# zir-vision/ProbPose_pytorch

Measured on AMD Instinct MI355X. Metric: person_crops_per_sec, higher is better.
Workload: dtype bf16

## Files before the change

### include/probpose_hip.h

```cpp
#ifndef PROBPOSE_HIP_H
#define PROBPOSE_HIP_H

#include <stddef.h>
#include <stdint.h>

#ifdef __cplusplus
extern "C" {
#endif

#define PP_F32 0
#define PP_BF16 1
#define PP_FP8 2

#define PP_MAX_RADIUS 9
#define PP_MAX_TAPS (2 * PP_MAX_RADIUS + 1)

#define PP_EPI_BIAS 1
#define PP_EPI_GELU 2
#define PP_EPI_RELU 4
#define PP_EPI_RESIDUAL 8
#define PP_EPI_OUT_F32 16
#define PP_EPI_ROWBIAS 32
#define PP_EPI_ROWSTATS 128
#define PP_EPI_LNFOLD 256
#define PP_EPI_OUT_FP8 512
#define PP_EPI_NOCLAMP 1024
#define PP_EPI_FUSE_FINAL 2048
#define PP_EPI_HEADMAJOR 4096
#define PP_EPI_HEATMAP 64

int pp_version(void);
const char *pp_last_error(void);
int pp_device_ok(void);

#define PP_DECODE_NO_WAVE 1
#define PP_DECODE_SCREEN 2
#define PP_DECODE_ALL_PIXEL 4
#define PP_DECODE_WAVE 16
size_t pp_decode_workspace_bytes(int B, int K, int H, int W);
int pp_decode_f32(const float *heatmaps, const float *prob, const float *vis,
                  const float *oks, const float *err, int B, int K, int H, int W,
                  const double *taps, const int *radius, double den_x, double den_y,
                  double in_w, double in_h, double *out_kpts, float *out_scores,
                  float *out_locs, float *out_aux, double *out_err, float *out_conv,
                  double *out_packed, void *workspace, int flags, void *stream);

typedef struct pp_gemm_args {
  const void *A; const void *W; void *C;
  const float *bias;
  const float *residual;
  const float *rowbias;
  const int32_t *rowoff;
  const int32_t *out_rowmap;
  int M, N, Kd;
  int lda, ldw, ldc;
  int seg_len;
  int rowbias_period;
  int batch;
  long long strideA, strideW, strideC, strideBias, strideRowoff, strideRowmap;
  int dtype;
  int epilogue;
  int hm_K, hm_HW;
  float hm_temperature;
  void *C2;
  int ldc2;
  float *stats_out;
  const float *stats_in;
  int stats_parts;
  const float *colsum;
  float ln_eps;
  int tile;
  float out_scale;
  int splitk;
  long long strideA_k, strideW_k, strideC_k, strideRowoff_k;
  const void *final_w;
  const float *final_b;
} pp_gemm_args;
int pp_gemm(const pp_gemm_args *args, void *stream);

int pp_layernorm(const float *x, const float *gamma, const float *beta, float eps,
                 int rows, int C, void *out, int dtype, void *stream);
int pp_layernorm_fp8(const float *x, const float *gamma, const float *beta, float eps,
                     int rows, int C, unsigned char *out, float inv_scale, void *stream);

int pp_attention(const void *qkv, void *out, int B, int N, int heads, int hd,
                 int dtype, void *stream);
int pp_attention_headmajor(const void *qkv, void *out, int B, int N, int heads, int hd, void *stream);
int pp_attention_fp8out(const void *qkv, unsigned char *out, int B, int N, int heads, int hd,
                        float inv_scale, void *stream);

int pp_qkv_attention_bf16(const void *h, const void *w_hm, const float *b_hm, void *out, int B, int heads, int C,
                          void *stream);

int pp_patchify(const float *x, void *out, int B, int H, int W, int patch, int dtype,
                void *stream);

int pp_maxpool_relu_sum(const float *x, int nsplit, long long split_stride, const float *bias, void *out, int B, int h,
                        int w, int C, int kh, int kw, int dtype, void *stream);

int pp_maxpool_relu(const void *x, void *out, int B, int h, int w, int C, int kh, int kw,
                    int dtype, void *stream);

int pp_final_heatmap(const void *x, const void *w, const float *bias, float *out, int B, int HW,
                     int Cin, int K, float temperature, int dtype, void *stream);

int pp_final_logits(const void *x, const void *w, const float *bias, float *out, int B, int HW,
                    int Cin, int K, float temperature, int dtype, void *stream);

int pp_sparsemax_rows(float *x, long long rows, int n, float scale, void *stream);

size_t pp_dark_decode_lds_bytes(int H, int W, int ksize);
int pp_dark_decode_f32(const float *heatmaps, int B, int K, int H, int W, const float *taps_host, int ksize,
                       double in_w, double in_h, double *out_kpts, float *out_scores, float *out_locs, void *stream);

int pp_aux_tail(const void *x, const void *w, const float *bias, float *out, int B, int C,
                int K, int dtype, void *stream);

int pp_tokens_to_nchw(const void *x, float *out, int B, int N, int C, int dtype, void *stream);
int pp_nchw_to_tokens(const float *x, void *out, int B, int C, int HW, int dtype, void *stream);

long long pp_frontend_plan_bytes(int n_boxes, const int *boxes_xyxy, int out_w, int out_h);
int pp_frontend_plan_build(int n_boxes, const int *boxes_xyxy, int out_w, int out_h, void *plan,
                           int *n_blocks_out, long long *lds_bytes_out);
int pp_frontend_crop_resize(const unsigned char *image, int img_w, int img_h, long long img_stride,
                            const void *plan_dev, int n_boxes, int n_blocks, long long lds_bytes,
                            int out_w, int out_h, float *out, void *stream);

#define PP_FRONTEND_SRC_ALIGN 4
#define PP_FRONTEND_SRC_PAD 4
long long pp_frontend_multi_plan_bytes(int n_boxes, const int *boxes_xyxy, int out_w, int out_h);
int pp_frontend_multi_plan_build(int n_boxes, const int *boxes_xyxy, const long long *sources, long long src_bytes,
                                 int out_w, int out_h, void *plan, int *n_blocks_out, long long *lds_bytes_out);
int pp_frontend_crop_resize_multi(const unsigned char *src, const void *plan_dev, int n_boxes, int n_blocks,
                                  long long lds_bytes, int out_w, int out_h, float *out, void *stream);

int pp_dataset_ground_truth(const float *kpts_raw, const double *boxes_xywh, int B, int K, int in_w, int in_h,
                            float scale_x, float scale_y, float *kpts_crop, float *kpts_hm, float *encode_visible,
                            unsigned char *in_image, unsigned char *keypoints_visible, float *keypoints_visibility,
                            void *stream);

int pp_augment_check(int n, const long long *sources, long long src_bytes, const double *warp,
                     const float *kp_affine, int K, const int *perm);
int pp_augment_warp(const unsigned char *src, const long long *sources, const double *warp, int n, int in_w,
                    int in_h, float *out, void *stream);
int pp_dataset_ground_truth_affine(const float *kpts_raw, const float *kp_affine, const int *perm, int B, int K,
                                   int in_w, int in_h, float scale_x, float scale_y, float *kpts_crop,
                                   float *kpts_hm, float *encode_visible, unsigned char *in_image,
                                   unsigned char *keypoints_visible, float *keypoints_visibility, void *stream);

#define PP_AUGMENT_POST_TILE_W 64
#define PP_AUGMENT_POST_TILE_H 16
int pp_augment_post_check(int n, const int *records, int in_w, int in_h, int filters);
int pp_augment_post(const float *in, const int *records, int n, int in_w, int in_h, int filters, float *out,
                    void *stream);

int pp_hflip_pair(const float *x, float *out, int B, int C, int H, int W, void *stream);
int pp_flip_merge(const float *heat2, const float *aux2, const int *perm, int B, int K, int H, int W,
                  float *heat_out, float *aux_out, void *stream);

int pp_encode_probmaps(const float *kpts_hm, const float *visible, const double *two_s, int B, int K, int H,
                       int W, float *heatmaps, float *weights, void *stream);

int pp_heatmap_argmax(const float *heatmaps, long long maps, int H, int W, float *locs, float *vals, void *stream);
int pp_pck_counts(const void *pred, const void *gt, int coord_f64, const unsigned char *mask, const double *norm,
                  const unsigned char *skip, double thr, int N, int K, int *counts, float *dist, void *stream);

// ... 222 lines not shown
```

### probpose_pytorch_amd/_lib.py

```python
from __future__ import annotations

import ctypes as C
import os
import threading

import numpy as np
import torch

_HERE = os.path.dirname(os.path.abspath(__file__))
LIB_PATH = os.path.join(_HERE, "lib", "libprobpose_hip.so")

PP_F32, PP_BF16, PP_FP8 = 0, 1, 2
PP_MAX_RADIUS = 9
PP_MAX_TAPS = 2 * PP_MAX_RADIUS + 1
EPI_BIAS, EPI_GELU, EPI_RELU, EPI_RESIDUAL, EPI_OUT_F32, EPI_ROWBIAS, EPI_HEATMAP = 1, 2, 4, 8, 16, 32, 64
DECODE_NO_WAVE, DECODE_SCREEN, DECODE_ALL_PIXEL, DECODE_WAVE = 1, 2, 4, 16
EPI_HEADMAJOR = 4096
EPI_OUT_FP8, EPI_NOCLAMP, EPI_FUSE_FINAL = 512, 1024, 2048

_lock = threading.Lock()
_lib = None


class HipExtensionError(RuntimeError):
    pass


class GemmArgs(C.Structure):
    _fields_ = [
        ("A", C.c_void_p), ("W", C.c_void_p), ("C", C.c_void_p),
        ("bias", C.c_void_p), ("residual", C.c_void_p), ("rowbias", C.c_void_p),
        ("rowoff", C.c_void_p), ("out_rowmap", C.c_void_p),
        ("M", C.c_int), ("N", C.c_int), ("Kd", C.c_int),
        ("lda", C.c_int), ("ldw", C.c_int), ("ldc", C.c_int),
        ("seg_len", C.c_int), ("rowbias_period", C.c_int), ("batch", C.c_int),
        ("strideA", C.c_longlong), ("strideW", C.c_longlong), ("strideC", C.c_longlong),
        ("strideBias", C.c_longlong), ("strideRowoff", C.c_longlong), ("strideRowmap", C.c_longlong),
        ("dtype", C.c_int), ("epilogue", C.c_int),
        ("hm_K", C.c_int), ("hm_HW", C.c_int), ("hm_temperature", C.c_float),
        ("C2", C.c_void_p), ("ldc2", C.c_int), ("stats_out", C.c_void_p), ("stats_in", C.c_void_p),
        ("stats_parts", C.c_int), ("colsum", C.c_void_p), ("ln_eps", C.c_float), ("tile", C.c_int),
        ("out_scale", C.c_float),
        ("splitk", C.c_int),
        ("strideA_k", C.c_longlong), ("strideW_k", C.c_longlong), ("strideC_k", C.c_longlong),
        ("strideRowoff_k", C.c_longlong),
        ("final_w", C.c_void_p), ("final_b", C.c_void_p),
    ]


class WgradArgs(C.Structure):
    _fields_ = [
        ("dY", C.c_void_p), ("dy_rowmap", C.c_void_p), ("ldd", C.c_longlong),
        ("A", C.c_void_p), ("rowoff", C.c_void_p), ("seg_len", C.c_int), ("lda", C.c_int),
        ("dW", C.c_void_p), ("lddw", C.c_longlong),
        ("dB", C.c_void_p),
        ("parts", C.c_void_p),
        ("M", C.c_int), ("N", C.c_int), ("Kd", C.c_int), ("batch", C.c_int),
        ("strideDY", C.c_longlong), ("strideA", C.c_longlong), ("strideRowoff", C.c_longlong),
        ("strideRowmap", C.c_longlong), ("strideDW", C.c_longlong), ("strideDB", C.c_longlong),
        ("dtype", C.c_int),
    ]


_vp, _i, _f, _d = C.c_void_p, C.c_int, C.c_float, C.c_double
_SIGNATURES = {
    "pp_version": (C.c_int, []),
    "pp_last_error": (C.c_char_p, []),
    "pp_device_ok": (C.c_int, []),
    "pp_decode_workspace_bytes": (C.c_size_t, [_i, _i, _i, _i]),
    "pp_decode_f32": (C.c_int, [_vp] * 5 + [_i] * 4 + [_vp, _vp] + [_d] * 4 + [_vp] * 8 + [_i, _vp]),
    "pp_gemm": (C.c_int, [C.POINTER(GemmArgs), _vp]),
    "pp_layernorm": (C.c_int, [_vp, _vp, _vp, _f, _i, _i, _vp, _i, _vp]),
    "pp_layernorm_fp8": (C.c_int, [_vp, _vp, _vp, _f, _i, _i, _vp, _f, _vp]),
    "pp_attention": (C.c_int, [_vp, _vp, _i, _i, _i, _i, _i, _vp]),
    "pp_attention_headmajor": (C.c_int, [_vp, _vp, _i, _i, _i, _i, _vp]),
    "pp_attention_fp8out": (C.c_int, [_vp, _vp, _i, _i, _i, _i, _f, _vp]),
    "pp_qkv_attention_bf16": (C.c_int, [_vp, _vp, _vp, _vp, _i, _i, _i, _vp]),
    "pp_patchify": (C.c_int, [_vp, _vp, _i, _i, _i, _i, _i, _vp]),
    "pp_maxpool_relu": (C.c_int, [_vp, _vp, _i, _i, _i, _i, _i, _i, _i, _vp]),
    "pp_maxpool_relu_sum": (C.c_int, [_vp, _i, C.c_longlong, _vp, _vp, _i, _i, _i, _i, _i, _i, _i, _vp]),
    "pp_final_heatmap": (C.c_int, [_vp, _vp, _vp, _vp, _i, _i, _i, _i, _f, _i, _vp]),
    "pp_final_logits": (C.c_int, [_vp, _vp, _vp, _vp, _i, _i, _i, _i, _f, _i, _vp]),
    "pp_sparsemax_rows": (C.c_int, [_vp, C.c_longlong, _i, _f, _vp]),
    "pp_dark_decode_lds_bytes": (C.c_size_t, [_i, _i, _i]),
    "pp_dark_decode_f32": (C.c_int, [_vp, _i, _i, _i, _i, _vp, _i, _d, _d, _vp, _vp, _vp, _vp]),
    "pp_aux_tail": (C.c_int, [_vp, _vp, _vp, _vp, _i, _i, _i, _i, _vp]),
    "pp_tokens_to_nchw": (C.c_int, [_vp, _vp, _i, _i, _i, _i, _vp]),
    "pp_nchw_to_tokens": (C.c_int, [_vp, _vp, _i, _i, _i, _i, _vp]),
    "pp_encode_probmaps": (C.c_int, [_vp, _vp, _vp, _i, _i, _i, _i, _vp, _vp, _vp]),
    "pp_heatmap_argmax": (C.c_int, [_vp, C.c_longlong, _i, _i, _vp, _vp, _vp]),
    "pp_pck_counts": (C.c_int, [_vp, _vp, _i, _vp, _vp, _vp, _d, _i, _i, _vp, _vp, _vp]),
    "pp_frontend_plan_bytes": (C.c_longlong, [_i, _vp, _i, _i]),
    "pp_frontend_plan_build": (C.c_int, [_i, _vp, _i, _i, _vp, C.POINTER(C.c_int), C.POINTER(C.c_longlong)]),
    "pp_frontend_crop_resize": (C.c_int, [_vp, _i, _i, C.c_longlong, _vp, _i, _i, C.c_longlong, _i, _i, _vp, _vp]),
    "pp_frontend_multi_plan_bytes": (C.c_longlong, [_i, _vp, _i, _i]),
    "pp_frontend_multi_plan_build": (C.c_int, [_i, _vp, _vp, C.c_longlong, _i, _i, _vp, C.POINTER(C.c_int),
                                               C.POINTER(C.c_longlong)]),
    "pp_frontend_crop_resize_multi": (C.c_int, [_vp, _vp, _i, _i, C.c_longlong, _i, _i, _vp, _vp]),
    "pp_dataset_ground_truth": (C.c_int, [_vp, _vp, _i, _i, _i, _i, _f, _f] + [_vp] * 7),
    "pp_augment_check": (C.c_int, [_i, _vp, C.c_longlong, _vp, _vp, _i, _vp]),
    "pp_augment_warp": (C.c_int, [_vp, _vp, _vp, _i, _i, _i, _vp, _vp]),
    "pp_dataset_ground_truth_affine": (C.c_int, [_vp, _vp, _vp, _i, _i, _i, _i, _f, _f] + [_vp] * 7),
    "pp_augment_post_check": (C.c_int, [_i, _vp, _i, _i, _i]),
    "pp_augment_post": (C.c_int, [_vp, _vp, _i, _i, _i, _i, _vp, _vp]),
    "pp_hflip_pair": (C.c_int, [_vp, _vp, _i, _i, _i, _i, _vp]),
    "pp_flip_merge": (C.c_int, [_vp, _vp, _vp, _i, _i, _i, _i, _vp, _vp, _vp]),
    "pp_oks_heatmap_loss": (C.c_int, [_vp, _vp, _vp, _i, _vp, C.c_longlong, C.c_longlong, _i, _i] + [_f] * 4
                            + [_i] * 4 + [_vp] * 5),
    "pp_probpose_loss_terms": (C.c_int, [_vp] * 10 + [_d, _i, _i, _i] + [_vp] * 6),
    "pp_oks_heatmap_loss_backward": (C.c_int, [_vp, _vp, _vp, _i, _vp, C.c_longlong, C.c_longlong, _i, _i]
                                     + [_f] * 4 + [_i, _vp] + [C.c_longlong] * 4 + [_i] * 4 + [_vp, _vp]),
    "pp_probpose_loss_grads": (C.c_int, [_vp] * 13 + [_i, _i] + [_vp] * 5),
    "pp_wgrad_workspace_floats": (C.c_longlong, [_i, _i, _i, _i]),
    "pp_wgrad_gemm": (C.c_int, [C.POINTER(WgradArgs), _vp]),
    "pp_bn_workspace_bytes": (C.c_longlong, [_i, _i]),
    "pp_bn_train_stats": (C.c_int, [_vp, C.c_longlong, _i, _i, _vp, _vp, _f, _f] + [_vp] * 8),
    "pp_bn_apply_relu": (C.c_int, [_vp, C.c_longlong, _i, _i, _vp, _vp, _vp, C.c_longlong, _i, _i, _vp]),
    "pp_bn_pool_relu": (C.c_int, [_vp, _i, _i, _i, _i, _i, _i, _vp, _vp, _vp, _vp, _i, _vp]),
    "pp_bn_train_backward": (C.c_int, [_vp, C.c_longlong, _vp, C.c_longlong, _i, _i] + [_vp] * 5
                             + [_i, _vp, _i, _i, _i, _i, _i, _vp, _vp, _vp, C.c_longlong, _i, _vp, _vp]),
    "pp_aux_tail_backward": (C.c_int, [_vp] * 4 + [_i, _i, _i] + [_vp] * 3 + [_i, _vp]),
    "pp_heat_clamp": (C.c_int, [_vp, _vp, C.c_longlong, _f, _vp]),
    "pp_heat_tail_backward": (C.c_int, [_vp, _vp, _i, _i, _i, _f, _i, _f, _vp, _i, _i, _vp]),
    "pp_layernorm_backward_workspace_bytes": (C.c_longlong, [_i, _i]),
    "pp_layernorm_backward": (C.c_int, [_vp, _vp, _f, _i, _i, _vp, C.c_longlong, _vp, _i, _vp, _i, _vp, _vp, _vp, _vp]),
    "pp_gelu_forward": (C.c_int, [_vp, C.c_longlong, _vp, _i, _vp]),
    "pp_gelu_backward": (C.c_int, [_vp, _vp, C.c_longlong, _vp, _i, _vp]),
    "pp_attention_backward_workspace_bytes": (C.c_longlong, [_i, _i, _i]),
    "pp_attention_backward": (C.c_int, [_vp] * 4 + [_i] * 5 + [_vp, _vp]),
    "pp_rows_period_sum": (C.c_int, [_vp, _i, _i, _i, _vp, _vp]),
    "pp_crop_rows_gather": (C.c_int, [_vp, _vp, _i, _i, _i, _i, _f, _vp, _i, _vp]),
    "pp_droppath_add": (C.c_int, [_vp, _vp, _vp, _i, _i, _i, _i, _f, _vp, _vp]),
    "pp_crop_rows_scatter_add": (C.c_int, [_vp, _vp, _i, _i, _i, _i, _vp, _vp, _i, _vp]),
    "pp_optim_table_bytes": (C.c_longlong, [_i, _vp, _i]),
    "pp_optim_table_build": (C.c_int, [_i] + [_vp] * 7 + [_i] + [_vp] * 3 + [_i, C.POINTER(C.c_int),
                                                                             C.POINTER(C.c_longlong)]),
    "pp_grad_sqnorm_partials": (C.c_int, [_vp, _i, _vp, _vp]),
    "pp_grad_norm_finish": (C.c_int, [_vp, _i, _i, _d, _i, _vp, _vp]),
    "pp_adamw_step": (C.c_int, [_vp, _i, _vp, _i, _vp]),
    "pp_ema_table_bytes": (C.c_longlong, [_i, _vp]),
    "pp_ema_table_build": (C.c_int, [_i] + [_vp] * 5 + [C.POINTER(C.c_int)]),
    "pp_ema_update": (C.c_int, [_vp, _i, _d, _vp]),
    "pp_cocoeval_oks": (C.c_int, [_i, _i] + [C.c_longlong] * 3 + [_vp] * 10),
    "pp_cocoeval_exoks": (C.c_int, [_i, _i] + [C.c_longlong] * 3 + [_vp] * 10 + [_d, _vp, _vp]),
    "pp_cocoeval_match": (C.c_int, [_i, _i, _i] + [C.c_longlong] * 3 + [_vp] * 13),
    "pp_cocoeval_accumulate": (C.c_int, [C.c_longlong, _i, _i, _i] + [_vp] * 10),
    "pp_posenms_rescore": (C.c_int, [C.c_longlong, _i, _vp, _vp, _d, _vp, _vp]),
    "pp_posenms": (C.c_int, [_i, _i, C.c_longlong] + [_vp] * 7 + [_i, _d, _d, _i] + [_vp] * 4),
    "pp_track_state_bytes": (C.c_longlong, [_i, _i]),
    "pp_track_oks": (C.c_int, [_i, _i, _i, C.c_longlong] + [_vp] * 7 + [_d, _vp, _vp]),
    "pp_track_assign": (C.c_int, [_i, _i, _i, C.c_longlong] + [_vp] * 5 + [_d, _i, _d, _d] + [_vp] * 6),
    "pp_track_assign_optimal": (C.c_int, [_i, _i, _i, C.c_longlong] + [_vp] * 5 + [_d, _i, _d, _d] + [_vp] * 7),
    "pp_track_oks_predicted": (C.c_int, [_i, _i, _i, C.c_longlong] + [_vp] * 7 + [_d, _d, _d, _vp, _vp]),
    "pp_track_assign_staged": (C.c_int, [_i, _i, _i, C.c_longlong] + [_vp] * 6 + [_d, _d, _d, _i, _d, _i, _i, _d, _d]
                               + [_vp] * 7),
    "pp_track_filter": (C.c_int, [_i, _i, C.c_longlong] + [_vp] * 4 + [_d] + [_vp] * 3 + [_i, _d, _d, _d, _vp, _vp]),
# ... 91 lines not shown
```

### probpose_pytorch_amd/csrc/pp_ops.hip

```cpp
#include <algorithm>

#include "pp_common.h"

namespace pp {

__device__ __forceinline__ float ln_sum4(float4 v) { return (v.x + v.y) + (v.z + v.w); }
__device__ __forceinline__ float ln_sqsum4(float4 v, float mean) {
  const float a = v.x - mean, b = v.y - mean, cc = v.z - mean, d = v.w - mean;
  return (a * a + b * b) + (cc * cc + d * d);
}
template <typename T>
__global__ __launch_bounds__(256) void layernorm_kernel(const float *__restrict__ x,
                                                        const float *__restrict__ gamma,
                                                        const float *__restrict__ beta, float eps,
                                                        int rows, int C, T *__restrict__ out, float qscale = 1.0f) {
  const int lane = threadIdx.x & 63;
  const int row = blockIdx.x * 4 + (threadIdx.x >> 6);
  if (row >= rows) return;
  const float *xr = x + (size_t)row * C;
  T *orow = out + (size_t)row * C;
  constexpr int MAXV = 8;
  if ((C & 3) == 0 && C <= MAXV * 256) {
    float4 v[MAXV];
    float s = 0.f;
#pragma unroll
    for (int i = 0; i < MAXV; ++i) {
      const int c = (i * 64 + lane) * 4;
      if (c < C) {
        v[i] = *reinterpret_cast<const float4 *>(xr + c);
        s += ln_sum4(v[i]);
      }
    }
    const float mean = wave_sum(s) / (float)C;
    float q = 0.f;
#pragma unroll
    for (int i = 0; i < MAXV; ++i) {
      const int c = (i * 64 + lane) * 4;
      if (c < C) {
        q += ln_sqsum4(v[i], mean);
      }
    }
    const float rstd = 1.0f / sqrtf(wave_sum(q) / (float)C + eps);
#pragma unroll
    for (int i = 0; i < MAXV; ++i) {
      const int c = (i * 64 + lane) * 4;
      if (c < C) {
        const float4 g = *reinterpret_cast<const float4 *>(gamma + c);
        const float4 b = *reinterpret_cast<const float4 *>(beta + c);
        const float o0 = (v[i].x - mean) * rstd * g.x + b.x, o1 = (v[i].y - mean) * rstd * g.y + b.y,
                    o2 = (v[i].z - mean) * rstd * g.z + b.z, o3 = (v[i].w - mean) * rstd * g.w + b.w;
        if constexpr (sizeof(T) == 4) {
          *reinterpret_cast<float4 *>(orow + c) = make_float4(o0, o1, o2, o3);
        } else if constexpr (sizeof(T) == 1) {
          *reinterpret_cast<unsigned *>(orow + c) = pack_fp8x4(o0 * qscale, o1 * qscale, o2 * qscale, o3 * qscale);
        } else {
          ushort4 pk;
          pk.x = f32_to_bf16(o0); pk.y = f32_to_bf16(o1); pk.z = f32_to_bf16(o2); pk.w = f32_to_bf16(o3);
          *reinterpret_cast<ushort4 *>(orow + c) = pk;
        }
      }
    }
    return;
  }
  float s = 0.f;
  for (int c = lane; c < C; c += 64) s += xr[c];
  const float mean = wave_sum(s) / (float)C;
  float q = 0.f;
  for (int c = lane; c < C; c += 64) {
    const float d = xr[c] - mean;
    q += d * d;
  }
  const float rstd = 1.0f / sqrtf(wave_sum(q) / (float)C + eps);
  if constexpr (sizeof(T) != 1)
    for (int c = lane; c < C; c += 64) Store<T>::st(orow + c, (xr[c] - mean) * rstd * gamma[c] + beta[c]);
}

template <typename T, int RPW, int NV>
__global__ __launch_bounds__(256) void layernorm_rows_kernel(const float *__restrict__ x,
                                                             const float *__restrict__ gamma,
                                                             const float *__restrict__ beta, float eps, int rows,
                                                             int C, T *__restrict__ out, float qscale) {
  const int lane = threadIdx.x & 63;
  const int row0 = (blockIdx.x * 4 + (threadIdx.x >> 6)) * RPW;
  if (row0 >= rows) return;
  float4 v[RPW][NV];
#pragma unroll
  for (int r = 0; r < RPW; ++r) {
    const float *xr = x + (size_t)min(row0 + r, rows - 1) * C;
#pragma unroll
    for (int i = 0; i < NV; ++i) {
      const int c = (i * 64 + lane) * 4;
      if (c < C) v[r][i] = *reinterpret_cast<const float4 *>(xr + c);
    }
  }
  float4 g[NV], bt[NV];
#pragma unroll
  for (int i = 0; i < NV; ++i) {
    const int c = (i * 64 + lane) * 4;
    if (c < C) {
      g[i] = *reinterpret_cast<const float4 *>(gamma + c);
      bt[i] = *reinterpret_cast<const float4 *>(beta + c);
    }
  }
#pragma unroll
  for (int r = 0; r < RPW; ++r) {
    float s = 0.f;
#pragma unroll
    for (int i = 0; i < NV; ++i) {
      const int c = (i * 64 + lane) * 4;
      if (c < C) s += ln_sum4(v[r][i]);
    }
    const float mean = wave_sum(s) / (float)C;
    float q = 0.f;
#pragma unroll
    for (int i = 0; i < NV; ++i) {
      const int c = (i * 64 + lane) * 4;
      if (c < C) {
        q += ln_sqsum4(v[r][i], mean);
      }
    }
    const float rstd = 1.0f / sqrtf(wave_sum(q) / (float)C + eps);
    if (row0 + r >= rows) continue;
    T *orow = out + (size_t)(row0 + r) * C;
#pragma unroll
    for (int i = 0; i < NV; ++i) {
      const int c = (i * 64 + lane) * 4;
      if (c < C) {
        const float o0 = (v[r][i].x - mean) * rstd * g[i].x + bt[i].x, o1 = (v[r][i].y - mean) * rstd * g[i].y + bt[i].y,
                    o2 = (v[r][i].z - mean) * rstd * g[i].z + bt[i].z, o3 = (v[r][i].w - mean) * rstd * g[i].w + bt[i].w;
        if constexpr (sizeof(T) == 4) {
          *reinterpret_cast<float4 *>(orow + c) = make_float4(o0, o1, o2, o3);
        } else if constexpr (sizeof(T) == 1) {
          *reinterpret_cast<unsigned *>(orow + c) = pack_fp8x4(o0 * qscale, o1 * qscale, o2 * qscale, o3 * qscale);
        } else {
          ushort4 pk;
          pk.x = f32_to_bf16(o0); pk.y = f32_to_bf16(o1); pk.z = f32_to_bf16(o2); pk.w = f32_to_bf16(o3);
          *reinterpret_cast<ushort4 *>(orow + c) = pk;
        }
      }
    }
  }
}

template <typename T>
static bool layernorm_rows_launch(const float *x, const float *gamma, const float *beta, float eps, int rows, int C,
                                  T *out, float qscale, hipStream_t s) {
  if ((C & 3) != 0 || C > 1280 || C <= 512 || rows < 2048) return false;
  const int want = (rows + 4095) / 4096;
  const int rpw = want >= 3 ? 3 : (want >= 2 ? 2 : 1);
  const int grid = cdiv(rows, 4 * rpw);
#define PP_LN_ROWS(RPW_, NV_)                                                                                     \
  hipLaunchKernelGGL((layernorm_rows_kernel<T, RPW_, NV_>), dim3(grid), dim3(256), 0, s, x, gamma, beta, eps, rows, C, \
                     out, qscale)
  if (C <= 768) {
    if (rpw == 3) PP_LN_ROWS(3, 3); else if (rpw == 2) PP_LN_ROWS(2, 3); else PP_LN_ROWS(1, 3);
  } else {
    if (rpw == 3) PP_LN_ROWS(3, 5); else if (rpw == 2) PP_LN_ROWS(2, 5); else PP_LN_ROWS(1, 5);
  }
#undef PP_LN_ROWS
  return true;
}

template <typename T>
__global__ __launch_bounds__(256) void patchify_kernel(const float *__restrict__ x, T *__restrict__ out,
                                                       int B, int H, int W, int p) {
  const int W4 = W >> 2;
  const long long total = (long long)B * 3 * H * W4;
  const int gw = W / p, gh = H / p;
  for (long long i = (long long)blockIdx.x * 256 + threadIdx.x; i < total; i += (long long)gridDim.x * 256) {
    const int xq = (int)(i % W4);
    long long t = i / W4;
    const int y = (int)(t % H);
    t /= H;
    const int c = (int)(t % 3);
    const int b = (int)(t / 3);
    const int x0 = xq * 4;
    const int gy = y / p, py = y - gy * p, gx = x0 / p, px = x0 - gx * p;
    if (gy >= gh || gx >= gw) continue;
    const float4 v = *reinterpret_cast<const float4 *>(x + (((size_t)b * 3 + c) * H + y) * W + x0);
    T *o = out + ((size_t)(b * gh + gy) * gw + gx) * (3 * p * p) + (c * p + py) * p + px;
    Store<T>::st(o + 0, v.x); Store<T>::st(o + 1, v.y); Store<T>::st(o + 2, v.z); Store<T>::st(o + 3, v.w);
  }
}

template <typename T>
__global__ __launch_bounds__(256) void maxpool_relu_kernel(const T *__restrict__ x, T *__restrict__ out,
                                                           int B, int h, int w, int C, int kh, int kw) {
  constexpr int VEC = 16 / (int)sizeof(T);
  const int oh = h / kh, ow = w / kw, CV = C / VEC;
  const long long total = (long long)B * oh * ow * CV;
  for (long long i = (long long)blockIdx.x * 256 + threadIdx.x; i < total; i += (long long)gridDim.x * 256) {
    const int cv = (int)(i % CV);
    long long t = i / CV;
    const int ox = (int)(t % ow);
    t /= ow;
    const int oy = (int)(t % oh);
    const int b = (int)(t / oh);
    float m[VEC];
#pragma unroll
    for (int e = 0; e < VEC; ++e) m[e] = 0.f;
    for (int dy = 0; dy < kh; ++dy)
      for (int dx = 0; dx < kw; ++dx) {
        const T *src = x + (((size_t)b * h + oy * kh + dy) * w + ox * kw + dx) * C + cv * VEC;
        const uint4 raw = *reinterpret_cast<const uint4 *>(src);
        const T *e8 = reinterpret_cast<const T *>(&raw);
#pragma unroll
        for (int e = 0; e < VEC; ++e) {
          const float f = Store<T>::ld(e8 + e);
          m[e] = (f > m[e] || f != f) ? f : m[e];
        }
      }
    uint4 pk;
    T *o8 = reinterpret_cast<T *>(&pk);
#pragma unroll
    for (int e = 0; e < VEC; ++e) Store<T>::st(o8 + e, m[e]);
    *reinterpret_cast<uint4 *>(out + (((size_t)b * oh + oy) * ow + ox) * C + cv * VEC) = pk;
  }
}

template <typename T>
__global__ __launch_bounds__(256) void maxpool_relu_sum_kernel(const float *__restrict__ x, int nsplit,
                                                               long long split_stride, const float *__restrict__ bias,
                                                               T *__restrict__ out, int B, int h, int w, int C, int kh,
                                                               int kw) {
  const int oh = h / kh, ow = w / kw, CV = C / 4;
  const long long total = (long long)B * oh * ow * CV;
  for (long long i = (long long)blockIdx.x * 256 + threadIdx.x; i < total; i += (long long)gridDim.x * 256) {
    const int cv = (int)(i % CV);
    long long t = i / CV;
    const int ox = (int)(t % ow);
    t /= ow;
    const int oy = (int)(t % oh);
    const int b = (int)(t / oh);
    const float4 bv = *reinterpret_cast<const float4 *>(bias + cv * 4);
    float m[4] = {0.f, 0.f, 0.f, 0.f};
    for (int dy = 0; dy < kh; ++dy)
      for (int dx = 0; dx < kw; ++dx) {
        const float *src = x + (((size_t)b * h + oy * kh + dy) * w + ox * kw + dx) * C + cv * 4;
        float4 a = *reinterpret_cast<const float4 *>(src);
        for (int sp = 1; sp < nsplit; ++sp) {
          const float4 q = *reinterpret_cast<const float4 *>(src + (size_t)sp * split_stride);
          a.x += q.x; a.y += q.y; a.z += q.z; a.w += q.w;
        }
        const float f[4] = {a.x + bv.x, a.y + bv.y, a.z + bv.z, a.w + bv.w};
#pragma unroll
        for (int e = 0; e < 4; ++e) m[e] = (f[e] > m[e] || f[e] != f[e]) ? f[e] : m[e];
      }
    T *o = out + (((size_t)b * oh + oy) * ow + ox) * C + cv * 4;
    if constexpr (sizeof(T) == 4) {
      *reinterpret_cast<float4 *>(o) = make_float4(m[0], m[1], m[2], m[3]);
    } else {
      ushort4 pk;
      pk.x = f32_to_bf16(m[0]); pk.y = f32_to_bf16(m[1]); pk.z = f32_to_bf16(m[2]); pk.w = f32_to_bf16(m[3]);
      *reinterpret_cast<ushort4 *>(o) = pk;
    }
  }
}

template <typename T>
__global__ __launch_bounds__(256) void aux_tail_kernel(const T *__restrict__ x, const T *__restrict__ w,
                                                       const float *__restrict__ bias,
                                                       float *__restrict__ out, int B, int C, int K,
                                                       int nbr, unsigned relu_mask) {
  const int lane = threadIdx.x & 63;
// ... 206 lines not shown
              const float4 kv = kr[d4];
              a = fmaf(q[4 * d4 + 0], kv.x, a);
              a = fmaf(q[4 * d4 + 1], kv.y, a);
              a = fmaf(q[4 * d4 + 2], kv.z, a);
              a = fmaf(q[4 * d4 + 3], kv.w, a);
            }
          } else {
            a = -__builtin_inff();
          }
          s[u] = a;
          gm = fmaxf(gm, a);
        }
        const float mn = fmaxf(m, gm);
        const float alpha = expf(m - mn);
        l *= alpha;
#pragma unroll
        for (int d = 0; d < HD; ++d) o[d] *= alpha;
#pragma unroll
        for (int u = 0; u < 8; ++u) {
          if (g + u < kc) {
            const float pu = expf(s[u] - mn);
            l += pu;
            const float4 *vr = reinterpret_cast<const float4 *>(Vs + (size_t)(g + u) * HD);
#pragma unroll
            for (int d4 = 0; d4 < HD / 4; ++d4) {
              const float4 vv = vr[d4];
              o[4 * d4 + 0] = fmaf(pu, vv.x, o[4 * d4 + 0]);
              o[4 * d4 + 1] = fmaf(pu, vv.y, o[4 * d4 + 1]);
              o[4 * d4 + 2] = fmaf(pu, vv.z, o[4 * d4 + 2]);
              o[4 * d4 + 3] = fmaf(pu, vv.w, o[4 * d4 + 3]);
            }
          }
        }
        m = mn;
      }
    }
    if (active) {
      const float inv = 1.0f / l;
      T *orow = out + ((size_t)b * N + qi) * C + h * HD;
#pragma unroll
      for (int d = 0; d < HD; ++d) Store<T>::st(orow + d, o[d] * inv);
    }
  }
}

template <typename T, int HD>
static int launch_attention_valu(const void *qkv, void *out, int B, int N, int heads, hipStream_t s) {
  int KC = (64 * 1024) / (2 * HD * 4);
  KC = (KC / 8) * 8;
  if (KC > N) KC = ((N + 7) / 8) * 8;
  const size_t lds = (size_t)2 * KC * HD * 4;
  int threads = ((N + 63) / 64) * 64;
  if (threads > 256) threads = 256;
  const float scale = 1.0f / sqrtf((float)HD);
  hipLaunchKernelGGL((attention_valu_kernel<T, HD>), dim3(B * heads), dim3(threads), lds, s,
                     (const T *)qkv, (T *)out, N, heads, scale, KC);
  PP_CHECK_LAUNCH("attention_valu_kernel");
  return 0;
}

template <typename T>
int attention_valu(const void *qkv, void *out, int B, int N, int heads, int hd, hipStream_t s) {
  switch (hd) {
    case 32: return launch_attention_valu<T, 32>(qkv, out, B, N, heads, s);
    case 64: return launch_attention_valu<T, 64>(qkv, out, B, N, heads, s);
    case 80: return launch_attention_valu<T, 80>(qkv, out, B, N, heads, s);
    default: return fail("pp_attention: head_dim %d not supported (32, 64, 80)", hd);
  }
}
template int attention_valu<float>(const void *, void *, int, int, int, int, hipStream_t);
template int attention_valu<bf16_t>(const void *, void *, int, int, int, int, hipStream_t);

static int grid_for(long long work_items) {
  long long g = (work_items + 255) / 256;
  if (g > 8192) g = 8192;
  if (g < 1) g = 1;
  return (int)g;
}

}

using namespace pp;

extern "C" int pp_layernorm(const float *x, const float *gamma, const float *beta, float eps, int rows,
                            int C, void *out, int dtype, void *stream) {
  PP_REQUIRE(rows >= 0 && C > 0, "pp_layernorm: bad shape");
  if (rows == 0) return 0;
  PP_REQUIRE(x && gamma && beta && out, "pp_layernorm: null pointer");
  hipStream_t s = (hipStream_t)stream;
  const int grid = cdiv(rows, 4);
  if (dtype == PP_BF16) {
    if (!layernorm_rows_launch<bf16_t>(x, gamma, beta, eps, rows, C, (bf16_t *)out, 1.0f, s))
      hipLaunchKernelGGL(layernorm_kernel<bf16_t>, dim3(grid), dim3(256), 0, s, x, gamma, beta, eps, rows, C,
                         (bf16_t *)out);
  } else if (dtype == PP_F32) {
    if (!layernorm_rows_launch<float>(x, gamma, beta, eps, rows, C, (float *)out, 1.0f, s))
      hipLaunchKernelGGL(layernorm_kernel<float>, dim3(grid), dim3(256), 0, s, x, gamma, beta, eps, rows, C,
                         (float *)out);
  } else {
    return fail("pp_layernorm: bad dtype %d", dtype);
  }
  PP_CHECK_LAUNCH("layernorm_kernel");
  return 0;
}

extern "C" int pp_layernorm_fp8(const float *x, const float *gamma, const float *beta, float eps, int rows, int C,
                                unsigned char *out, float inv_scale, void *stream) {
  PP_REQUIRE(rows >= 0 && C > 0 && (C & 3) == 0 && C <= 2048, "pp_layernorm_fp8: C must be a multiple of 4, <= 2048");
  PP_REQUIRE(inv_scale > 0.f, "pp_layernorm_fp8: inv_scale must be positive");
  if (rows == 0) return 0;
  PP_REQUIRE(x && gamma && beta && out, "pp_layernorm_fp8: null pointer");
  if (!layernorm_rows_launch<unsigned char>(x, gamma, beta, eps, rows, C, out, inv_scale, (hipStream_t)stream))
    hipLaunchKernelGGL(layernorm_kernel<unsigned char>, dim3(cdiv(rows, 4)), dim3(256), 0, (hipStream_t)stream, x, gamma,
                       beta, eps, rows, C, out, inv_scale);
  PP_CHECK_LAUNCH("layernorm_kernel<fp8>");
  return 0;
}

extern "C" int pp_patchify(const float *x, void *out, int B, int H, int W, int patch, int dtype,
                           void *stream) {
  PP_REQUIRE(B >= 0 && H > 0 && W > 0 && patch > 0, "pp_patchify: bad shape");
  if (B == 0) return 0;
  PP_REQUIRE(x && out, "pp_patchify: null pointer");
  PP_REQUIRE(W % 4 == 0 && patch % 4 == 0, "pp_patchify: W and patch must be multiples of 4");
  hipStream_t s = (hipStream_t)stream;
  const int grid = grid_for((long long)B * 3 * H * (W / 4));
  if (dtype == PP_BF16)
    hipLaunchKernelGGL(patchify_kernel<bf16_t>, dim3(grid), dim3(256), 0, s, x, (bf16_t *)out, B, H, W, patch);
  else if (dtype == PP_F32)
    hipLaunchKernelGGL(patchify_kernel<float>, dim3(grid), dim3(256), 0, s, x, (float *)out, B, H, W, patch);
  else
    return fail("pp_patchify: bad dtype %d", dtype);
  PP_CHECK_LAUNCH("patchify_kernel");
  return 0;
}

extern "C" int pp_maxpool_relu(const void *x, void *out, int B, int h, int w, int C, int kh, int kw,
                               int dtype, void *stream) {
  PP_REQUIRE(B >= 0 && h > 0 && w > 0 && C > 0 && kh > 0 && kw > 0, "pp_maxpool_relu: bad shape");
  PP_REQUIRE(h / kh > 0 && w / kw > 0, "pp_maxpool_relu: window %dx%d larger than input %dx%d", kh, kw, h, w);
  if (B == 0) return 0;
  PP_REQUIRE(x && out, "pp_maxpool_relu: null pointer");
  hipStream_t s = (hipStream_t)stream;
  const int vec = dtype == PP_BF16 ? 8 : 4;
  PP_REQUIRE(C % vec == 0, "pp_maxpool_relu: C=%d must be a multiple of %d", C, vec);
  const int grid = grid_for((long long)B * (h / kh) * (w / kw) * (C / vec));
  if (dtype == PP_BF16)
    hipLaunchKernelGGL(maxpool_relu_kernel<bf16_t>, dim3(grid), dim3(256), 0, s, (const bf16_t *)x,
                       (bf16_t *)out, B, h, w, C, kh, kw);
  else if (dtype == PP_F32)
    hipLaunchKernelGGL(maxpool_relu_kernel<float>, dim3(grid), dim3(256), 0, s, (const float *)x,
                       (float *)out, B, h, w, C, kh, kw);
  else
    return fail("pp_maxpool_relu: bad dtype %d", dtype);
  PP_CHECK_LAUNCH("maxpool_relu_kernel");
  return 0;
}

extern "C" int pp_aux_tail(const void *x, const void *w, const float *bias, float *out, int B, int C,
                           int K, int dtype, void *stream) {
  PP_REQUIRE(B >= 0 && C > 0 && K > 0, "pp_aux_tail: bad shape");
  if (B == 0) return 0;
  PP_REQUIRE(x && w && bias && out, "pp_aux_tail: null pointer");
  hipStream_t s = (hipStream_t)stream;
  const int nbr = 4;
  const unsigned relu_mask = 1u << 3;
  const int grid = cdiv((long long)nbr * B * K, 4);
  if (dtype == PP_BF16)
    hipLaunchKernelGGL(aux_tail_kernel<bf16_t>, dim3(grid), dim3(256), 0, s, (const bf16_t *)x,
                       (const bf16_t *)w, bias, out, B, C, K, nbr, relu_mask);
  else if (dtype == PP_F32)
    hipLaunchKernelGGL(aux_tail_kernel<float>, dim3(grid), dim3(256), 0, s, (const float *)x,
                       (const float *)w, bias, out, B, C, K, nbr, relu_mask);
  else
    return fail("pp_aux_tail: bad dtype %d", dtype);
  PP_CHECK_LAUNCH("aux_tail_kernel");
  return 0;
}

extern "C" int pp_maxpool_relu_sum(const float *x, int nsplit, long long split_stride, const float *bias, void *out,
                                   int B, int h, int w, int C, int kh, int kw, int dtype, void *stream) {
  PP_REQUIRE(B >= 0 && h > 0 && w > 0 && C > 0 && kh > 0 && kw > 0 && nsplit >= 1, "pp_maxpool_relu_sum: bad shape");
  PP_REQUIRE(h / kh > 0 && w / kw > 0, "pp_maxpool_relu_sum: window %dx%d larger than input %dx%d", kh, kw, h, w);
  if (B == 0) return 0;
  PP_REQUIRE(x && bias && out, "pp_maxpool_relu_sum: null pointer");
  PP_REQUIRE(C % 4 == 0 && split_stride % 4 == 0, "pp_maxpool_relu_sum: C and the split stride must be multiples of 4");
  hipStream_t s = (hipStream_t)stream;
  const int grid = grid_for((long long)B * (h / kh) * (w / kw) * (C / 4));
  if (dtype == PP_BF16)
    hipLaunchKernelGGL(maxpool_relu_sum_kernel<bf16_t>, dim3(grid), dim3(256), 0, s, x, nsplit, split_stride, bias,
                       (bf16_t *)out, B, h, w, C, kh, kw);
  else if (dtype == PP_F32)
    hipLaunchKernelGGL(maxpool_relu_sum_kernel<float>, dim3(grid), dim3(256), 0, s, x, nsplit, split_stride, bias,
                       (float *)out, B, h, w, C, kh, kw);
  else
    return fail("pp_maxpool_relu_sum: bad dtype %d", dtype);
  PP_CHECK_LAUNCH("maxpool_relu_sum_kernel");
  return 0;
}

template <bool CLAMP>
static int final_heatmap_launch(const void *x, const void *w, const float *bias, float *out, int B, int HW,
                                int Cin, int K, float temperature, int dtype, void *stream) {
  PP_REQUIRE(B >= 0 && HW > 0 && Cin > 0 && K > 0 && temperature != 0.f, "pp_final_heatmap: bad shape");
  if (B == 0) return 0;
  PP_REQUIRE(x && w && bias && out, "pp_final_heatmap: null pointer");
  PP_REQUIRE(dtype == PP_BF16 || dtype == PP_F32, "pp_final_heatmap: bad dtype %d", dtype);
  const int es = dtype == PP_BF16 ? 2 : 4, vec = 16 / es;
  PP_REQUIRE(Cin % vec == 0, "pp_final_heatmap: Cin=%d must be a multiple of %d", Cin, vec);
  const long long M = (long long)B * HW;
  PP_REQUIRE(M < (1ll << 31), "pp_final_heatmap: too many rows");
  if (dtype == PP_BF16 && HW % 16 == 0 && Cin % 32 == 0 && Cin <= 32 * FHM_MAXKS && K <= 144 &&
      ((uintptr_t)x & 15) == 0 && ((uintptr_t)w & 15) == 0 && ((uintptr_t)out & 15) == 0) {
    const int nt = cdiv(K, 16), tiles = (int)(M / 16);
    const int grid = (int)std::min<long long>(cdiv(tiles, 4), 256 * 2);
// ... 79 lines not shown
```

Baseline: 17490.

## Add pipelined multi-row layernorm form and vectorize patchify stores

Replaces the multi-row layernorm kernel with a persistent-capable pipelined kernel that double-buffers row loads across groups, and exposes a tunable entry point for rows per group and workgroups per CU. The defaults (one row per group, no grid cap) make the default path roughly a one-row-per-wave launch, unlike the previous adaptive 1-3 rows per wave. Patchify is rewritten to use unsigned index maths, a linear input address, and vectorized 4-element stores when the output is aligned. The goals are fewer scattered scalar stores and cheaper index division; the layernorm default change may shift occupancy and latency hiding.

New measurement: 17360. About the same (-0.7%).

```diff
diff --git a/include/probpose_hip.h b/include/probpose_hip.h
--- a/include/probpose_hip.h
+++ b/include/probpose_hip.h
@@ -82,6 +82,8 @@
                  int rows, int C, void *out, int dtype, void *stream);
 int pp_layernorm_fp8(const float *x, const float *gamma, const float *beta, float eps,
                      int rows, int C, unsigned char *out, float inv_scale, void *stream);
+int pp_layernorm_form(const float *x, const float *gamma, const float *beta, float eps, int rows, int C, void *out,
+                      int dtype, float qscale, int rows_per_group, int wg_per_cu, void *stream);
 
 int pp_attention(const void *qkv, void *out, int B, int N, int heads, int hd,
                  int dtype, void *stream);
diff --git a/probpose_pytorch_amd/_lib.py b/probpose_pytorch_amd/_lib.py
--- a/probpose_pytorch_amd/_lib.py
+++ b/probpose_pytorch_amd/_lib.py
@@ -72,6 +72,7 @@
     "pp_gemm": (C.c_int, [C.POINTER(GemmArgs), _vp]),
     "pp_layernorm": (C.c_int, [_vp, _vp, _vp, _f, _i, _i, _vp, _i, _vp]),
     "pp_layernorm_fp8": (C.c_int, [_vp, _vp, _vp, _f, _i, _i, _vp, _f, _vp]),
+    "pp_layernorm_form": (C.c_int, [_vp, _vp, _vp, _f, _i, _i, _vp, _i, _f, _i, _i, _vp]),
     "pp_attention": (C.c_int, [_vp, _vp, _i, _i, _i, _i, _i, _vp]),
     "pp_attention_headmajor": (C.c_int, [_vp, _vp, _i, _i, _i, _i, _vp]),
     "pp_attention_fp8out": (C.c_int, [_vp, _vp, _i, _i, _i, _i, _f, _vp]),
diff --git a/probpose_pytorch_amd/csrc/pp_ops.hip b/probpose_pytorch_amd/csrc/pp_ops.hip
--- a/probpose_pytorch_amd/csrc/pp_ops.hip
+++ b/probpose_pytorch_amd/csrc/pp_ops.hip
@@ -8,6 +8,27 @@
 __device__ __forceinline__ float ln_sqsum4(float4 v, float mean) {
   const float a = v.x - mean, b = v.y - mean, cc = v.z - mean, d = v.w - mean;
   return (a * a + b * b) + (cc * cc + d * d);
+}
+__device__ __forceinline__ float ln_centred_scaled(float v, float mean, float rstd) {
+  float d, r;
+  asm("v_sub_f32 %0, %1, %2" : "=v"(d) : "v"(v), "v"(mean));
+  asm("v_mul_f32 %0, %1, %2" : "=v"(r) : "v"(d), "v"(rstd));
+  return r;
+}
+template <typename T>
+__device__ __forceinline__ void ln_store4(float4 v, float mean, float rstd, float4 g, float4 b, float qscale,
+                                          T *__restrict__ dst) {
+  const float o0 = ln_centred_scaled(v.x, mean, rstd) * g.x + b.x, o1 = ln_centred_scaled(v.y, mean, rstd) * g.y + b.y,
+              o2 = ln_centred_scaled(v.z, mean, rstd) * g.z + b.z, o3 = ln_centred_scaled(v.w, mean, rstd) * g.w + b.w;
+  if constexpr (sizeof(T) == 4) {
+    *reinterpret_cast<float4 *>(dst) = make_float4(o0, o1, o2, o3);
+  } else if constexpr (sizeof(T) == 1) {
+    *reinterpret_cast<unsigned *>(dst) = pack_fp8x4(o0 * qscale, o1 * qscale, o2 * qscale, o3 * qscale);
+  } else {
+    ushort4 pk;
+    pk.x = f32_to_bf16(o0); pk.y = f32_to_bf16(o1); pk.z = f32_to_bf16(o2); pk.w = f32_to_bf16(o3);
+    *reinterpret_cast<ushort4 *>(dst) = pk;
+  }
 }
 template <typename T>
 __global__ __launch_bounds__(256) void layernorm_kernel(const float *__restrict__ x,
@@ -47,17 +68,7 @@
       if (c < C) {
         const float4 g = *reinterpret_cast<const float4 *>(gamma + c);
         const float4 b = *reinterpret_cast<const float4 *>(beta + c);
-        const float o0 = (v[i].x - mean) * rstd * g.x + b.x, o1 = (v[i].y - mean) * rstd * g.y + b.y,
-                    o2 = (v[i].z - mean) * rstd * g.z + b.z, o3 = (v[i].w - mean) * rstd * g.w + b.w;
-        if constexpr (sizeof(T) == 4) {
-          *reinterpret_cast<float4 *>(orow + c) = make_float4(o0, o1, o2, o3);
-        } else if constexpr (sizeof(T) == 1) {
-          *reinterpret_cast<unsigned *>(orow + c) = pack_fp8x4(o0 * qscale, o1 * qscale, o2 * qscale, o3 * qscale);
-        } else {
-          ushort4 pk;
-          pk.x = f32_to_bf16(o0); pk.y = f32_to_bf16(o1); pk.z = f32_to_bf16(o2); pk.w = f32_to_bf16(o3);
-          *reinterpret_cast<ushort4 *>(orow + c) = pk;
-        }
+        ln_store4<T>(v[i], mean, rstd, g, b, qscale, orow + c);
       }
     }
     return;
@@ -75,24 +86,69 @@
     for (int c = lane; c < C; c += 64) Store<T>::st(orow + c, (xr[c] - mean) * rstd * gamma[c] + beta[c]);
 }
 
-template <typename T, int RPW, int NV>
-__global__ __launch_bounds__(256) void layernorm_rows_kernel(const float *__restrict__ x,
+template <typename T, int NV>
+__device__ __forceinline__ void ln_row(const float4 (&v)[NV], const float4 (&g)[NV], const float4 (&bt)[NV], int lane,
+                                       int C, float eps, float qscale, T *__restrict__ orow, bool store) {
+  float s = 0.f;
+#pragma unroll
+  for (int i = 0; i < NV; ++i) {
+    const int c = (i * 64 + lane) * 4;
+    if (c < C) s += ln_sum4(v[i]);
+  }
+  const float mean = wave_sum(s) / (float)C;
+  float q = 0.f;
+#pragma unroll
+  for (int i = 0; i < NV; ++i) {
+    const int c = (i * 64 + lane) * 4;
+    if (c < C) {
+      q += ln_sqsum4(v[i], mean);
+    }
+  }
+  const float rstd = 1.0f / sqrtf(wave_sum(q) / (float)C + eps);
+  if (!store) return;
+#pragma unroll
+  for (int i = 0; i < NV; ++i) {
+    const int c = (i * 64 + lane) * 4;
+    if (c < C) {
+      ln_store4<T>(v[i], mean, rstd, g[i], bt[i], qscale, orow + c);
+    }
+  }
+}
+
+template <int RPG, int NV>
+__device__ __forceinline__ void ln_load_group(float4 (&v)[RPG][NV], const float *__restrict__ x, int row0, int rows,
+                                              int C, int lane) {
+#pragma unroll
+  for (int r = 0; r < RPG; ++r) {
+    const float *xr = x + (size_t)min(row0 + r, rows - 1) * C;
+#pragma unroll
+    for (int i = 0; i < NV; ++i) {
+      const int c = (i * 64 + lane) * 4;
+      if (c < C) v[r][i] = *reinterpret_cast<const float4 *>(xr + c);
+    }
+  }
+}
+
+template <typename T, int RPG, int NV>
+__device__ __forceinline__ void ln_group(const float4 (&v)[RPG][NV], const float4 (&g)[NV], const float4 (&bt)[NV],
+                                         int lane, int row0, int rows, int C, float eps, float qscale,
+                                         T *__restrict__ out) {
+#pragma unroll
+  for (int r = 0; r < RPG; ++r)
+    ln_row<T, NV>(v[r], g, bt, lane, C, eps, qscale, out + (size_t)min(row0 + r, rows - 1) * C, row0 + r < rows);
+}
+
+template <typename T, int RPG, int NV, bool LOOP>
+__global__ __launch_bounds__(256) void layernorm_pipe_kernel(const float *__restrict__ x,
                                                              const float *__restrict__ gamma,
                                                              const float *__restrict__ beta, float eps, int rows,
                                                              int C, T *__restrict__ out, float qscale) {
   const int lane = threadIdx.x & 63;
-  const int row0 = (blockIdx.x * 4 + (threadIdx.x >> 6)) * RPW;
-  if (row0 >= rows) return;
-  float4 v[RPW][NV];
-#pragma unroll
-  for (int r = 0; r < RPW; ++r) {
-    const float *xr = x + (size_t)min(row0 + r, rows - 1) * C;
-#pragma unroll
-    for (int i = 0; i < NV; ++i) {
-      const int c = (i * 64 + lane) * 4;
-      if (c < C) v[r][i] = *reinterpret_cast<const float4 *>(xr + c);
-    }
-  }
+  const int waves = gridDim.x * 4, groups = (rows + RPG - 1) / RPG;
+  int grp = blockIdx.x * 4 + (threadIdx.x >> 6);
+  if (grp >= groups) return;
+  float4 a[RPG][NV];
+  ln_load_group<RPG, NV>(a, x, grp * RPG, rows, C, lane);
   float4 g[NV], bt[NV];
 #pragma unroll
   for (int i = 0; i < NV; ++i) {
@@ -102,84 +158,85 @@
       bt[i] = *reinterpret_cast<const float4 *>(beta + c);
     }
   }
-#pragma unroll
-  for (int r = 0; r < RPW; ++r) {
-    float s = 0.f;
-#pragma unroll
-    for (int i = 0; i < NV; ++i) {
-      const int c = (i * 64 + lane) * 4;
-      if (c < C) s += ln_sum4(v[r][i]);
-    }
-    const float mean = wave_sum(s) / (float)C;
-    float q = 0.f;
-#pragma unroll
-    for (int i = 0; i < NV; ++i) {
-      const int c = (i * 64 + lane) * 4;
-      if (c < C) {
-        q += ln_sqsum4(v[r][i], mean);
-      }
-    }
-    const float rstd = 1.0f / sqrtf(wave_sum(q) / (float)C + eps);
-    if (row0 + r >= rows) continue;
-    T *orow = out + (size_t)(row0 + r) * C;
-#pragma unroll
-    for (int i = 0; i < NV; ++i) {
-      const int c = (i * 64 + lane) * 4;
-      if (c < C) {
-        const float o0 = (v[r][i].x - mean) * rstd * g[i].x + bt[i].x, o1 = (v[r][i].y - mean) * rstd * g[i].y + bt[i].y,
-                    o2 = (v[r][i].z - mean) * rstd * g[i].z + bt[i].z, o3 = (v[r][i].w - mean) * rstd * g[i].w + bt[i].w;
-        if constexpr (sizeof(T) == 4) {
-          *reinterpret_cast<float4 *>(orow + c) = make_float4(o0, o1, o2, o3);
-        } else if constexpr (sizeof(T) == 1) {
-          *reinterpret_cast<unsigned *>(orow + c) = pack_fp8x4(o0 * qscale, o1 * qscale, o2 * qscale, o3 * qscale);
-        } else {
-          ushort4 pk;
-          pk.x = f32_to_bf16(o0); pk.y = f32_to_bf16(o1); pk.z = f32_to_bf16(o2); pk.w = f32_to_bf16(o3);
-          *reinterpret_cast<ushort4 *>(orow + c) = pk;
-        }
-      }
-    }
-  }
-}
+  if constexpr (!LOOP) {
+    ln_group<T, RPG, NV>(a, g, bt, lane, grp * RPG, rows, C, eps, qscale, out);
+    return;
+  }
+  float4 b[RPG][NV];
+  for (;;) {
+    bool more = groups - grp > waves;
+    if (more) ln_load_group<RPG, NV>(b, x, (grp + waves) * RPG, rows, C, lane);
+    ln_group<T, RPG, NV>(a, g, bt, lane, grp * RPG, rows, C, eps, qscale, out);
+    if (!more) break;
+    grp += waves;
+    more = groups - grp > waves;
+    if (more) ln_load_group<RPG, NV>(a, x, (grp + waves) * RPG, rows, C, lane);
+    ln_group<T, RPG, NV>(b, g, bt, lane, grp * RPG, rows, C, eps, qscale, out);
+    if (!more) break;
+    grp += waves;
+  }
+}
+
+static bool layernorm_pipe_domain(int rows, int C) { return (C & 3) == 0 && C > 512 && C <= 1280 && rows >= 2048; }
 
 template <typename T>
-static bool layernorm_rows_launch(const float *x, const float *gamma, const float *beta, float eps, int rows, int C,
-                                  T *out, float qscale, hipStream_t s) {
-  if ((C & 3) != 0 || C > 1280 || C <= 512 || rows < 2048) return false;
-  const int want = (rows + 4095) / 4096;
-  const int rpw = want >= 3 ? 3 : (want >= 2 ? 2 : 1);
-  const int grid = cdiv(rows, 4 * rpw);
-#define PP_LN_ROWS(RPW_, NV_)                                                                                     \
-  hipLaunchKernelGGL((layernorm_rows_kernel<T, RPW_, NV_>), dim3(grid), dim3(256), 0, s, x, gamma, beta, eps, rows, C, \
-                     out, qscale)
+static int layernorm_pipe_launch(const float *x, const float *gamma, const float *beta, float eps, int rows, int C,
+                                 T *out, float qscale, int rpg, int wg_per_cu, hipStream_t s) {
+  int ncu = 0;
+  if (int rc = cu_count(&ncu)) return rc;
+  const int round = cdiv(cdiv(rows, rpg), 4);
+  const int grid = wg_per_cu > 0 ? std::min(wg_per_cu * ncu, round) : round;
+#define PP_LN_PIPE(RPG_, NV_)                                                                                     \
+  do {                                                                                                            \
+    if (grid == round)                                                                                            \
+      hipLaunchKernelGGL((layernorm_pipe_kernel<T, RPG_, NV_, false>), dim3(grid), dim3(256), 0, s, x, gamma, beta, eps, \
+                         rows, C, out, qscale);                                                                   \
+    else                                                                                                          \
+      hipLaunchKernelGGL((layernorm_pipe_kernel<T, RPG_, NV_, true>), dim3(grid), dim3(256), 0, s, x, gamma, beta, eps, \
+                         rows, C, out, qscale);                                                                   \
+  } while (0)
   if (C <= 768) {
-    if (rpw == 3) PP_LN_ROWS(3, 3); else if (rpw == 2) PP_LN_ROWS(2, 3); else PP_LN_ROWS(1, 3);
+    if (rpg == 3) PP_LN_PIPE(3, 3); else if (rpg == 2) PP_LN_PIPE(2, 3); else PP_LN_PIPE(1, 3);
   } else {
-    if (rpw == 3) PP_LN_ROWS(3, 5); else if (rpw == 2) PP_LN_ROWS(2, 5); else PP_LN_ROWS(1, 5);
-  }
-#undef PP_LN_ROWS
-  return true;
-}
-
-template <typename T>
+    if (rpg == 3) PP_LN_PIPE(3, 5); else if (rpg == 2) PP_LN_PIPE(2, 5); else PP_LN_PIPE(1, 5);
+  }
+#undef PP_LN_PIPE
+  PP_CHECK_LAUNCH("layernorm_pipe_kernel");
+  return 0;
+}
+
+constexpr int LN_PIPE_RPG = 1, LN_PIPE_WG_PER_CU = 0;
+
+template <typename T, bool VEC>
 __global__ __launch_bounds__(256) void patchify_kernel(const float *__restrict__ x, T *__restrict__ out,
                                                        int B, int H, int W, int p) {
-  const int W4 = W >> 2;
+  const unsigned W4 = W >> 2;
   const long long total = (long long)B * 3 * H * W4;
-  const int gw = W / p, gh = H / p;
+  const bool small = total <= 0xffffffffll;
+  const unsigned gw = W / p, gh = H / p;
   for (long long i = (long long)blockIdx.x * 256 + threadIdx.x; i < total; i += (long long)gridDim.x * 256) {
-    const int xq = (int)(i % W4);
-    long long t = i / W4;
-    const int y = (int)(t % H);
-    t /= H;
-    const int c = (int)(t % 3);
-    const int b = (int)(t / 3);
-    const int x0 = xq * 4;
-    const int gy = y / p, py = y - gy * p, gx = x0 / p, px = x0 - gx * p;
+    unsigned row, xq;
+    if (small) {
+      row = (unsigned)i / W4;
+      xq = (unsigned)i - row * W4;
+    } else {
+      row = (unsigned)(i / W4);
+      xq = (unsigned)(i - (long long)row * W4);
+    }
+    const unsigned bc = row / (unsigned)H, y = row - bc * H;
+    const unsigned b = bc / 3u, c = bc - 3u * b;
+    const unsigned x0 = xq * 4;
+    const unsigned gy = y / (unsigned)p, py = y - gy * p, gx = x0 / (unsigned)p, px = x0 - gx * p;
     if (gy >= gh || gx >= gw) continue;
-    const float4 v = *reinterpret_cast<const float4 *>(x + (((size_t)b * 3 + c) * H + y) * W + x0);
+    const float4 v = *reinterpret_cast<const float4 *>(x + (size_t)i * 4);
     T *o = out + ((size_t)(b * gh + gy) * gw + gx) * (3 * p * p) + (c * p + py) * p + px;
-    Store<T>::st(o + 0, v.x); Store<T>::st(o + 1, v.y); Store<T>::st(o + 2, v.z); Store<T>::st(o + 3, v.w);
+    if constexpr (!VEC) {
+      Store<T>::st(o + 0, v.x); Store<T>::st(o + 1, v.y); Store<T>::st(o + 2, v.z); Store<T>::st(o + 3, v.w);
+    } else if constexpr (sizeof(T) == 4) {
+      *reinterpret_cast<float4 *>(o) = v;
+    } else {
+      *reinterpret_cast<uint2 *>(o) = make_uint2(pack_bf16x2(v.x, v.y), pack_bf16x2(v.z, v.w));
+    }
   }
 }
 
@@ -552,26 +609,25 @@
 
 using namespace pp;
 
+template <typename T>
+static int layernorm_dispatch(const float *x, const float *gamma, const float *beta, float eps, int rows, int C, T *out,
+                              float qscale, hipStream_t s) {
+  if (layernorm_pipe_domain(rows, C))
+    return layernorm_pipe_launch<T>(x, gamma, beta, eps, rows, C, out, qscale, LN_PIPE_RPG, LN_PIPE_WG_PER_CU, s);
+  hipLaunchKernelGGL(layernorm_kernel<T>, dim3(cdiv(rows, 4)), dim3(256), 0, s, x, gamma, beta, eps, rows, C, out, qscale);
+  PP_CHECK_LAUNCH("layernorm_kernel");
+  return 0;
+}
+
 extern "C" int pp_layernorm(const float *x, const float *gamma, const float *beta, float eps, int rows,
                             int C, void *out, int dtype, void *stream) {
   PP_REQUIRE(rows >= 0 && C > 0, "pp_layernorm: bad shape");
   if (rows == 0) return 0;
   PP_REQUIRE(x && gamma && beta && out, "pp_layernorm: null pointer");
   hipStream_t s = (hipStream_t)stream;
-  const int grid = cdiv(rows, 4);
-  if (dtype == PP_BF16) {
-    if (!layernorm_rows_launch<bf16_t>(x, gamma, beta, eps, rows, C, (bf16_t *)out, 1.0f, s))
-      hipLaunchKernelGGL(layernorm_kernel<bf16_t>, dim3(grid), dim3(256), 0, s, x, gamma, beta, eps, rows, C,
-                         (bf16_t *)out);
-  } else if (dtype == PP_F32) {
-    if (!layernorm_rows_launch<float>(x, gamma, beta, eps, rows, C, (float *)out, 1.0f, s))
-      hipLaunchKernelGGL(layernorm_kernel<float>, dim3(grid), dim3(256), 0, s, x, gamma, beta, eps, rows, C,
-                         (float *)out);
-  } else {
-    return fail("pp_layernorm: bad dtype %d", dtype);
-  }
-  PP_CHECK_LAUNCH("layernorm_kernel");
-  return 0;
+  if (dtype == PP_BF16) return layernorm_dispatch<bf16_t>(x, gamma, beta, eps, rows, C, (bf16_t *)out, 1.0f, s);
+  if (dtype == PP_F32) return layernorm_dispatch<float>(x, gamma, beta, eps, rows, C, (float *)out, 1.0f, s);
+  return fail("pp_layernorm: bad dtype %d", dtype);
 }
 
 extern "C" int pp_layernorm_fp8(const float *x, const float *gamma, const float *beta, float eps, int rows, int C,
@@ -580,11 +636,27 @@
   PP_REQUIRE(inv_scale > 0.f, "pp_layernorm_fp8: inv_scale must be positive");
   if (rows == 0) return 0;
   PP_REQUIRE(x && gamma && beta && out, "pp_layernorm_fp8: null pointer");
-  if (!layernorm_rows_launch<unsigned char>(x, gamma, beta, eps, rows, C, out, inv_scale, (hipStream_t)stream))
-    hipLaunchKernelGGL(layernorm_kernel<unsigned char>, dim3(cdiv(rows, 4)), dim3(256), 0, (hipStream_t)stream, x, gamma,
-                       beta, eps, rows, C, out, inv_scale);
-  PP_CHECK_LAUNCH("layernorm_kernel<fp8>");
-  return 0;
+  return layernorm_dispatch<unsigned char>(x, gamma, beta, eps, rows, C, out, inv_scale, (hipStream_t)stream);
+}
+
+extern "C" int pp_layernorm_form(const float *x, const float *gamma, const float *beta, float eps, int rows, int C,
+                                 void *out, int dtype, float qscale, int rows_per_group, int wg_per_cu, void *stream) {
+  PP_REQUIRE(rows > 0 && layernorm_pipe_domain(rows, C), "pp_layernorm_form: rows=%d C=%d outside the multi-row form",
+             rows, C);
+  PP_REQUIRE(rows_per_group >= 1 && rows_per_group <= 3 && wg_per_cu >= 0 && wg_per_cu <= 16,
+             "pp_layernorm_form: bad launch shape rows_per_group=%d wg_per_cu=%d", rows_per_group, wg_per_cu);
+  PP_REQUIRE(x && gamma && beta && out, "pp_layernorm_form: null pointer");
+  hipStream_t s = (hipStream_t)stream;
+  if (dtype == PP_BF16)
+    return layernorm_pipe_launch<bf16_t>(x, gamma, beta, eps, rows, C, (bf16_t *)out, 1.0f, rows_per_group, wg_per_cu, s);
+  if (dtype == PP_F32)
+    return layernorm_pipe_launch<float>(x, gamma, beta, eps, rows, C, (float *)out, 1.0f, rows_per_group, wg_per_cu, s);
+  if (dtype == PP_FP8) {
+    PP_REQUIRE(qscale > 0.f, "pp_layernorm_form: qscale must be positive");
+    return layernorm_pipe_launch<unsigned char>(x, gamma, beta, eps, rows, C, (unsigned char *)out, qscale,
+                                                rows_per_group, wg_per_cu, s);
+  }
+  return fail("pp_layernorm_form: bad dtype %d", dtype);
 }
 
 extern "C" int pp_patchify(const float *x, void *out, int B, int H, int W, int patch, int dtype,
@@ -595,12 +667,20 @@
   PP_REQUIRE(W % 4 == 0 && patch % 4 == 0, "pp_patchify: W and patch must be multiples of 4");
   hipStream_t s = (hipStream_t)stream;
   const int grid = grid_for((long long)B * 3 * H * (W / 4));
+#define PP_PATCHIFY(T_)                                                                                              \
+  do {                                                                                                               \
+    if ((uintptr_t)out % (4 * sizeof(T_)) == 0)                                                                      \
+      hipLaunchKernelGGL((patchify_kernel<T_, true>), dim3(grid), dim3(256), 0, s, x, (T_ *)out, B, H, W, patch);    \
+    else                                                                                                             \
+      hipLaunchKernelGGL((patchify_kernel<T_, false>), dim3(grid), dim3(256), 0, s, x, (T_ *)out, B, H, W, patch);   \
+  } while (0)
   if (dtype == PP_BF16)
-    hipLaunchKernelGGL(patchify_kernel<bf16_t>, dim3(grid), dim3(256), 0, s, x, (bf16_t *)out, B, H, W, patch);
+    PP_PATCHIFY(bf16_t);
   else if (dtype == PP_F32)
-    hipLaunchKernelGGL(patchify_kernel<float>, dim3(grid), dim3(256), 0, s, x, (float *)out, B, H, W, patch);
+    PP_PATCHIFY(float);
   else
     return fail("pp_patchify: bad dtype %d", dtype);
+#undef PP_PATCHIFY
   PP_CHECK_LAUNCH("patchify_kernel");
   return 0;
 }
```
